# ysig/diff-mining

Measured on AMD Instinct MI355X. Metric: typicality-scored images/sec/node (512px, 10 t×2 prompts), higher is better.
Workload: dtype f16

## Files before the change

diff-mining_amd/build.py:

```python
from __future__ import annotations

import hashlib
import os
import subprocess
import sys
import time
from concurrent.futures import ThreadPoolExecutor

HERE = os.path.dirname(os.path.abspath(__file__))
CSRC = os.path.join(HERE, "csrc")
OBJ = os.path.join(CSRC, "build")
LIBDIR = os.path.join(HERE, "lib")
LIB = os.path.join(LIBDIR, "libdm_engine.so")
SOURCES = ["igemm.hip", "igemm_pers.hip", "igemm_pers_ln.hip", "igemm_pers_part.hip", "igemm_pers_ws.hip", "igemm_ws.hip", "igemm_pers_sc.hip", "igemm_sc.hip", "igemm_pers_tr.hip", "igemm_pers_up.hip", "igemm_ko.hip", "igemm_ln.hip", "igemm64.hip", "igemm_splitk.hip", "attention.hip", "attention_pipe.hip", "attention_qk32.hip", "attention_d160.hip", "attention_pp.hip", "attention_pipe80.hip", "attention_cross.hip", "resize.hip", "norm.hip", "misc.hip", "conv_out.hip", "vae.hip", "clip.hip", "f32_gemm.hip", "f32_ops.hip", "unet_f32.hip", "probe_peak.hip", "engine.hip"]
HEADERS = [os.path.join(CSRC, "dm_kernels.h"), os.path.join(CSRC, "f32_kernels.h"), os.path.join(CSRC, "arena.h"), os.path.join(CSRC, "igemm_tile.h"), os.path.join(CSRC, "igemm_pers_tile.h"), os.path.join(os.path.dirname(HERE), "include", "dm_engine.h")]
FLAGS = ["--offload-arch=gfx950", "-O3", "-std=c++17", "-fPIC", "-ffp-contract=off", "-Wno-unused-result",
         "-mllvm", "-amdgpu-mfma-vgpr-form=1"]


def _hipcc() -> str:
    for c in (os.environ.get("HIPCC"), "/opt/rocm/bin/hipcc", "hipcc"):
        if c and (os.path.isabs(c) and os.path.exists(c) or not os.path.isabs(c)):
            return c
    raise RuntimeError("hipcc not found")


def _read(path: str) -> bytes:
    with open(path, "rb") as f:
        return f.read()


_hipcc_id_cache = {}


def _hipcc_id(hipcc: str) -> bytes:
    if hipcc not in _hipcc_id_cache:
        r = subprocess.run([hipcc, "--version"], capture_output=True, text=True)
        _hipcc_id_cache[hipcc] = (r.stdout + r.stderr).encode()
    return _hipcc_id_cache[hipcc]


def tu_digest(src: str, hipcc: str) -> str:
    h = hashlib.sha256()
    h.update(_read(os.path.join(CSRC, src)))
    for hd in HEADERS:
        h.update(hd.encode())
        h.update(_read(hd))
    h.update(" ".join(FLAGS).encode())
    h.update(_hipcc_id(hipcc))
    return h.hexdigest()


def _stamp(obj: str) -> str:
    return obj + ".sha256"


def _tu_stale(src: str, obj: str, hipcc: str) -> bool:
    if not os.path.exists(obj) or not os.path.exists(_stamp(obj)):
        return True
    return _read(_stamp(obj)).decode().strip() != tu_digest(src, hipcc)


def build(force: bool = False, verbose: bool = False) -> str:
    os.makedirs(OBJ, exist_ok=True)
    os.makedirs(LIBDIR, exist_ok=True)
    hipcc = _hipcc()
    force = force or os.environ.get("DM_BUILD_FORCE", "0") not in ("", "0")
    t0 = time.time()
    jobs = []
    for src in SOURCES:
        o = os.path.join(OBJ, src.replace(".hip", ".o"))
        if force or _tu_stale(src, o, hipcc):
            jobs.append((src, o, [hipcc] + FLAGS + ["-c", os.path.join(CSRC, src), "-o", o]))

    def run(cmd):
        if verbose:
            print(" ".join(cmd), file=sys.stderr)
        r = subprocess.run(cmd, capture_output=True, text=True)
        if r.returncode != 0:
            raise RuntimeError("hipcc failed:\n" + " ".join(cmd) + "\n" + r.stdout + r.stderr)

    def compile_one(job):
        src, o, cmd = job
        if os.path.exists(_stamp(o)):
            os.remove(_stamp(o))
        run(cmd)
        with open(_stamp(o), "w") as f:
            f.write(tu_digest(src, hipcc) + "\n")
    with ThreadPoolExecutor(max_workers=min(8, os.cpu_count() or 1)) as ex:
        list(ex.map(compile_one, jobs))
    objs = [os.path.join(OBJ, s.replace(".hip", ".o")) for s in SOURCES]
    link_digest = hashlib.sha256("".join(_read(_stamp(o)).decode() for o in objs).encode()).hexdigest()
    linked = False
    if force or jobs or not os.path.exists(LIB) or not os.path.exists(_stamp(LIB)) or _read(_stamp(LIB)).decode().strip() != link_digest:
        run([hipcc, "--offload-arch=gfx950", "-shared", "-fPIC", "-o", LIB] + objs)
        with open(_stamp(LIB), "w") as f:
            f.write(link_digest + "\n")
        linked = True
    print(f"dm_engine build: compiled {len(jobs)}/{len(SOURCES)} TUs"
          f"{' (' + ', '.join(j[0] for j in jobs) + ')' if jobs and len(jobs) < len(SOURCES) else ''}, "
          f"{'linked' if linked else 'link up to date'} {os.path.relpath(LIB, os.path.dirname(HERE))} "
          f"[{link_digest[:12]}] in {time.time() - t0:.1f} s{' (forced)' if force else ''}", file=sys.stderr, flush=True)
    return LIB


if __name__ == "__main__":
    print(build(force="--force" in sys.argv, verbose="-v" in sys.argv))
```

diff-mining_amd/csrc/attention.hip:

```cpp
#include "dm_kernels.h"
#include <cstdlib>

namespace dm {

typedef _Float16 half8 __attribute__((ext_vector_type(8)));
typedef _Float16 half4 __attribute__((ext_vector_type(4)));
typedef float floatx4 __attribute__((ext_vector_type(4)));
typedef unsigned int u32x4 __attribute__((ext_vector_type(4)));
typedef unsigned int u32x2 __attribute__((ext_vector_type(2)));

namespace {

constexpr int KT = 64;
constexpr int NT = 256;
constexpr float RESCALE_THR = 8.0f;

__device__ __attribute__((aligned(256))) unsigned char g_attn_zero[256];
typedef const __attribute__((address_space(1))) void* gptr_t;
typedef __attribute__((address_space(3))) void* lptr_t;

template <int D, int QF>
__global__ __launch_bounds__(NT, (D > 80 ? 1 : 2))
void attn_kernel(AttnParams p) {
    constexpr int DP = ((D + 31) / 32) * 32, DV = ((D + 15) / 16) * 16;
// ... 142 lines not shown
            mx = __builtin_fmaxf(mx, __shfl_xor(mx, 32));
            if constexpr (FOLD) {
                float ps = 0.f;
                if (first || __builtin_amdgcn_ballot_w64(mx > RESCALE_THR) != 0ull) {
                    const float delta = first ? mx : __builtin_fmaxf(mx, 0.f);
                    const float alpha = first ? 0.f : __builtin_amdgcn_exp2f(-delta);
                    m_run[jq] += delta;
                    if (!LONES) l_run[jq] *= alpha;
#pragma unroll
                    for (int e = 0; e < EF; ++e) oacc[e][jq] *= alpha;
                    if (lg == LGX) {
                        const f16 mh = (f16)m_run[jq];
                        const f16 ml = (f16)(m_run[jq] - (float)mh);
                        qf[jq][SX][0] = -mh; qf[jq][SX][1] = -ml;
                    }
#pragma unroll
                    for (int f = 0; f < 4; ++f)
#pragma unroll
                        for (int r = 0; r < 4; ++r) {
                            const float pv = __builtin_amdgcn_exp2f(sacc[f][jq][r] - delta);
                            if (!LONES) ps += pv;
                            pb[jq][f >> 1][(f & 1) * 4 + r] = (f16)pv;
                        }
                } else {
#pragma unroll
                    for (int f = 0; f < 4; ++f)
#pragma unroll
                        for (int r = 0; r < 4; ++r) {
                            const float pv = __builtin_amdgcn_exp2f(sacc[f][jq][r]);
                            if (!LONES) ps += pv;
                            pb[jq][f >> 1][(f & 1) * 4 + r] = (f16)pv;
                        }
                }
                if (!LONES) l_run[jq] += ps;
            } else {
                const float mxs = mx * sc;
                if (__builtin_amdgcn_ballot_w64(mxs > m_run[jq] + RESCALE_THR) != 0ull) {
                    const float m_new = __builtin_fmaxf(m_run[jq], mxs);
                    const float alpha = __builtin_amdgcn_exp2f(m_run[jq] - m_new);
                    m_run[jq] = m_new;
                    l_run[jq] *= alpha;
#pragma unroll
                    for (int e = 0; e < EF; ++e) oacc[e][jq] *= alpha;
                }
                const float m_use = m_run[jq];
                float ps = 0.f;
#pragma unroll
                for (int f = 0; f < 4; ++f)
#pragma unroll
                    for (int r = 0; r < 4; ++r) {
                        const float pv = __builtin_amdgcn_exp2f(__builtin_fmaf(sacc[f][jq][r], sc, -m_use));
                        ps += pv;
                        pb[jq][f >> 1][(f & 1) * 4 + r] = (f16)pv;
                    }
                l_run[jq] += ps;
            }
        }
        constexpr int NB = (EF <= 5) ? 1 : 2;
#pragma unroll
        for (int bt = 0; bt < NB; ++bt) {
            u32x2 vraw[2 / NB][EF][2];
#pragma unroll
            for (int s2 = 0; s2 < 2 / NB; ++s2)
#pragma unroll
                for (int e = 0; e < EF; ++e)
#pragma unroll
                    for (int hh = 0; hh < 2; ++hh) {
                        const int ss = bt * (2 / NB) + s2;
                        const unsigned a = (unsigned)(size_t)(kt + voff[e] + (2 * ss + hh) * vstep[e]);
                        asm volatile("ds_read_b64_tr_b16 %0, %1" : "=v"(vraw[s2][e][hh]) : "v"(a) : "memory");
                    }
            asm volatile("s_waitcnt lgkmcnt(0)" ::: "memory");
            __builtin_amdgcn_sched_barrier(0);
#pragma unroll
            for (int s2 = 0; s2 < 2 / NB; ++s2)
#pragma unroll
                for (int e = 0; e < EF; ++e) {
                    const int ss = bt * (2 / NB) + s2;
                    half8 va;
                    __builtin_memcpy(&va, &vraw[s2][e][0], 8);
                    __builtin_memcpy(reinterpret_cast<char*>(&va) + 8, &vraw[s2][e][1], 8);
#pragma unroll
                    for (int jq = 0; jq < QF; ++jq)
                        oacc[e][jq] = __builtin_amdgcn_mfma_f32_16x16x32_f16(va, pb[jq][ss], oacc[e][jq], 0, 0, 0);
                }
        }
    };

    const int ntiles = (p.Tk + KT - 1) / KT;
    auto compute_tile = [&](int cur, int k0) __attribute__((always_inline)) {
        if (k0 + 64 > p.Tk) compute(cur, k0, true, k0 == 0); else compute(cur, k0, false, k0 == 0);
    };
    issue(0, 0);
    for (int t = 0; t < ntiles; ++t) {
        const int cur = t & 1;
        asm volatile("s_waitcnt vmcnt(0)" ::: "memory");
        __syncthreads();
        if (t + 1 < ntiles) issue(cur ^ 1, (t + 1) * KT);
        compute_tile(cur, t * KT);
    }

#pragma unroll
    for (int jq = 0; jq < QF; ++jq) {
        float l;
        if constexpr (LONES) {
            l = __shfl(oacc[EX][jq][0], (VLX << 4) | l15);
        } else {
            l = l_run[jq];
            l += __shfl_xor(l, 16);
            l += __shfl_xor(l, 32);
        }
        const float inv = 1.0f / l;
        const int q = q0 + 16 * jq + l15;
        if (q >= p.Tq) continue;
#pragma unroll
        for (int e = 0; e < EF; ++e) {
            const int d = 16 * e + 4 * lg;
            if (d < D) {
                const half4 o = half4{(f16)(oacc[e][jq][0] * inv), (f16)(oacc[e][jq][1] * inv),
                                      (f16)(oacc[e][jq][2] * inv), (f16)(oacc[e][jq][3] * inv)};
                *reinterpret_cast<half4*>(Ob + (size_t)q * p.ldo + d) = o;
            }
        }
    }
}

template <int D, int QF>
hipError_t launch_t(const AttnParams& p, hipStream_t s) {
    constexpr int QBLK = 64 * QF;
    dim3 grid((p.Tq + QBLK - 1) / QBLK, p.heads, p.B), block(NT);
    const size_t lds = 2 * (2 * (size_t)KT * D * 2 + 64);
    static std::atomic<uint64_t> attr_seen{0};
    if (first_use_on_device(attr_seen)) {
        (void)hipFuncSetAttribute((const void*)attn_kernel<D, QF>, hipFuncAttributeMaxDynamicSharedMemorySize, (int)lds);
    }
    launch_timed((attn_kernel<D, QF>), grid, block, lds, s, p);
    return hipGetLastError();
}

}

hipError_t launch_attention_pipe(const AttnParams& p, hipStream_t s);
bool attention_pipe_supports(const AttnParams& p);
hipError_t launch_attention_pipe80(const AttnParams& p, hipStream_t s);
bool attention_pipe80_supports(const AttnParams& p);
hipError_t launch_attention_cross(const AttnParams& p, hipStream_t s);
bool attention_cross_supports(const AttnParams& p);
hipError_t launch_attention_d160(const AttnParams& p, hipStream_t s);
bool attention_d160_supports(const AttnParams& p);
hipError_t launch_attention_d160_cross(const AttnParams& p, hipStream_t s);
bool attention_d160_cross_supports(const AttnParams& p);
hipError_t launch_attention_qk32(const AttnParams& p, hipStream_t s);
bool attention_qk32_supports(const AttnParams& p);
hipError_t launch_attention_pp(const AttnParams& p, int variant, hipStream_t s);
bool attention_pp_supports(const AttnParams& p);

hipError_t launch_attention(const AttnParams& p, hipStream_t s) {
    if (p.Tq <= 0 || p.Tk <= 0 || p.B <= 0) return hipErrorInvalidValue;
    if (option(OPT_ATTN_CROSS) && attention_cross_supports(p)) return launch_attention_cross(p, s);
    if (option(OPT_ATTN_CROSS) && attention_d160_cross_supports(p)) return launch_attention_d160_cross(p, s);
    const int pipe = option(OPT_ATTN_PIPE);
    if (p.q_mod > 0) {
        switch (p.D) { case 40: return launch_t<40, 2>(p, s); case 80: return launch_t<80, 2>(p, s); case 160: return launch_t<160, 2>(p, s); default: return hipErrorInvalidValue; }
    }
    if ((pipe == 10 || pipe == 12) && attention_pp_supports(p)) return launch_attention_pp(p, pipe, s);
    if (pipe == 5 && attention_qk32_supports(p)) return launch_attention_qk32(p, s);
#ifdef DM_ATTN_PP_ABLATE
    if (pipe >= 4 && pipe != 9 && attention_pp_supports(p)) return launch_attention_pp(p, pipe, s);
#endif
    if (pipe == 1 && p.Tk >= 8192 && attention_pp_supports(p) && (long long)((p.Tq + 383) / 384) * 384 * 50 <= 51LL * p.Tq)
        return launch_attention_pp(p, 12, s);
    if (pipe == 1 && attention_qk32_supports(p)) return launch_attention_qk32(p, s);
    if (pipe && attention_pipe_supports(p)) return launch_attention_pipe(p, s);
    if ((pipe == 1 || pipe >= 3) && attention_pipe80_supports(p)) return launch_attention_pipe80(p, s);
    if ((pipe == 1 || pipe == 5) && attention_d160_supports(p)) return launch_attention_d160(p, s);
    switch (p.D) {
        case 40: return launch_t<40, 2>(p, s);
        case 80: return launch_t<80, 2>(p, s);
        case 160: return launch_t<160, 2>(p, s);
        default: return hipErrorInvalidValue;
    }
}

}
```

diff-mining_amd/csrc/engine.hip:

```cpp
#include "../../include/dm_engine.h"
#include "dm_kernels.h"
#include "arena.h"

#include <cmath>
#include <cstdio>
#include <cstdlib>
#include <cstring>
#include <map>
#include <string>
#include <vector>

using namespace dm;

namespace {

thread_local std::string g_create_error;
}
namespace dm { thread_local LaunchTimer* g_launch_timer = nullptr; }
namespace {

constexpr int NB = 4;
const int BOC[NB] = {320, 640, 1280, 1280};
constexpr int LAYERS = 2;
constexpr int CTX_DIM = 768;
// ... 1055 lines not shown
        F.free(h);
        DM_TRY(F.alloc(&a, 1, 1, M, CL_H));
        if (!dry) DM_HIP(e, launch_clip_attention(qkv.p, n, CL_T, CL_HEADS, a.p, s));
        F.free(qkv);
        DM_TRY(F.dense(L.o, a, nullptr, &x, EPI_PLAIN, &x1));
        F.free(a); F.free(x);
        DM_TRY(F.layernorm(L.ln2, x1, &h));
        DM_TRY(F.dense(L.fc1, h, nullptr, nullptr, EPI_PLAIN, &f));
        F.free(h);
        if (!dry) DM_HIP(e, launch_quick_gelu(f.p, (long long)M * CL_F, s));
        DM_TRY(F.dense(L.fc2, f, nullptr, &x1, EPI_PLAIN, &x2));
        F.free(f); F.free(x1);
        x = x2;
    }
    Tensor y;
    DM_TRY(F.layernorm(c.final_ln, x, &y));
    F.free(x);
    if (!dry) {
        if (out16) DM_HIP(e, hipMemcpyAsync(out16, y.p, (size_t)M * CL_H * sizeof(f16), hipMemcpyDeviceToDevice, s));
        if (out32) DM_HIP(e, launch_f16_to_f32(y.p, out32, (long long)M * CL_H, s));
    }
    F.free(y);
    return 0;
}

void drop_graphs(dm_engine* e) {
    for (auto& g : e->graphs) (void)hipGraphExecDestroy(g.exec);
    e->graphs.clear();
}

template <class RunFn>
int ensure_arena_for(dm_engine* e, hipStream_t s, const std::vector<long long>& key, RunFn run_dry) {
    size_t need;
    if (e->opt_epoch != options_epoch()) {
        if (!e->graphs.empty()) { DM_HIP(e, hipStreamSynchronize(s)); drop_graphs(e); }
        e->arena_need.clear(); e->graph_seen.clear();
        e->opt_epoch = options_epoch();
    }
    auto it = e->arena_need.find(key);
    if (it != e->arena_need.end()) need = it->second;
    else {
        e->arena.reset((size_t)1 << 60, true);
        char* keep = e->arena_base;
        e->arena_base = nullptr;
        int rc = run_dry();
        e->arena_base = keep;
        if (rc) return rc;
        need = e->arena.peak;
        e->arena_need[key] = need;
        ++e->n_dry_runs;
    }
    if (need > e->arena_cap) {
        DM_HIP(e, hipStreamSynchronize(s));
        drop_graphs(e);
        if (e->arena_base) DM_HIP(e, hipFree(e->arena_base));
        e->arena_base = nullptr; e->arena_cap = 0;
        const size_t cap = need + (need >> 4);
        DM_MALLOC(e, &e->arena_base, cap);
        e->arena_cap = cap;
    }
    e->arena.reset(e->arena_cap, false);
    return 0;
}

std::vector<long long> fwd_key(const FwdArgs& A) {
    return {0, A.B, A.H, A.W, A.n_cond, A.up_ft_index, A.add_noise ? 1 : 0, A.loss ? 1 : 0, A.pred ? 1 : 0, A.feat ? 1 : 0,
            A.feat_mean ? 1 : 0, option(OPT_LN_FOLD), option(OPT_IGEMM_SPLITK), option(OPT_LN_INKERNEL), option(OPT_GN_FOLD), option(OPT_SC_FOLD), option(OPT_FF_FOLD), option(OPT_UP_FOLD), option(OPT_Q_ONCE), option(OPT_GN_EPI), option(OPT_CONV_OUT_ROWS), option(OPT_GN_SKIP)};
}

int ensure_arena(dm_engine* e, const FwdArgs& A, hipStream_t s) {
    return ensure_arena_for(e, s, fwd_key(A), [&]() { return run_forward(e, A, s, true); });
}

int reserve_prompts(dm_engine* e, int n_prompts, hipStream_t s) {
    if (n_prompts <= e->kv_capacity) return 0;
    int cap = e->kv_capacity > 0 ? 2 * e->kv_capacity : 16;
    if (cap < n_prompts) cap = n_prompts;
    DM_HIP(e, hipStreamSynchronize(s));
    drop_graphs(e);
    for (int l = 0; l < e->n_tf; ++l) {
        if (e->kv_cache[l]) DM_HIP(e, hipFree(e->kv_cache[l]));
        e->kv_cache[l] = nullptr;
        DM_MALLOC(e, &e->kv_cache[l], (size_t)cap * CTX_LEN * 2 * e->tfs[l]->c * sizeof(f16));
    }
    e->kv_capacity = cap;
    e->n_prompts = 0;
    return 0;
}

int run_forward_graphed(dm_engine* e, const FwdArgs& A, hipStream_t s) {
    if (!option(OPT_GRAPH) || e->prof || s == nullptr) return run_forward(e, A, s, false);
    std::vector<long long> key = fwd_key(A);
    for (const void* q : {A.x, (const void*)A.x_index, A.eps, (const void*)A.t, (const void*)A.slots, (const void*)A.loss,
                          (const void*)A.pred, (const void*)A.feat, (const void*)A.feat_mean, (const void*)s})
        key.push_back((long long)(size_t)q);
    for (long long v : {(long long)A.latent_f32, (long long)A.out_stride, (long long)A.out_off, (long long)A.ensemble, (long long)e->n_prompts})
        key.push_back(v);
    for (int o = 0; o < OPT_COUNT; ++o) key.push_back(option((Option)o));
    for (auto& g : e->graphs)
        if (g.key == key) {
            g.stamp = ++e->graph_stamp;
            ++e->n_graph_launches;
            DM_HIP(e, hipGraphLaunch(g.exec, s));
            return 0;
        }
    if (e->graph_seen.size() > 256) e->graph_seen.clear();
    if (e->graph_seen[key]++ == 0) return run_forward(e, A, s, false);
    hipGraph_t graph = nullptr;
    DM_HIP(e, hipStreamBeginCapture(s, hipStreamCaptureModeThreadLocal));
    const int rc = run_forward(e, A, s, false);
    const hipError_t ec = hipStreamEndCapture(s, &graph);
    if (rc) { if (graph) (void)hipGraphDestroy(graph); return rc; }
    if (ec != hipSuccess || !graph) DM_FAIL(e, "hipStreamEndCapture failed: %s", hipGetErrorString(ec));
    hipGraphExec_t exec = nullptr;
    const hipError_t ei = hipGraphInstantiate(&exec, graph, nullptr, nullptr, 0);
    (void)hipGraphDestroy(graph);
    if (ei != hipSuccess) DM_FAIL(e, "hipGraphInstantiate failed: %s", hipGetErrorString(ei));
    if (e->graphs.size() >= 8) {
        size_t old = 0;
        for (size_t i = 1; i < e->graphs.size(); ++i) if (e->graphs[i].stamp < e->graphs[old].stamp) old = i;
        (void)hipGraphExecDestroy(e->graphs[old].exec);
        e->graphs.erase(e->graphs.begin() + old);
    }
    e->graphs.push_back({key, exec, ++e->graph_stamp});
    ++e->n_graph_captures; ++e->n_graph_launches;
    DM_HIP(e, hipGraphLaunch(exec, s));
    return 0;
}

int max_chunk(int h, int w) {
    const long long px = (long long)h * w;
    static long long budget = -1;
    if (budget < 0) { const char* e = getenv("DM_CHUNK"); budget = e ? atoll(e) : 160; if (budget < 1) budget = 1; }
    long long b = (budget * 4096) / px;
    if (b < 1) b = 1;
    return (int)b;
}

}

namespace dm {

namespace {
struct OptDef { const char* name; const char* env; int def; };
const OptDef kOpts[OPT_COUNT] = {
    {"igemm_big", "DM_IGEMM_BIG", -1}, {"igemm_splitk", "DM_IGEMM_SPLITK", 1},
    {"ln_fold", "DM_LN_FOLD", 1}, {"attn_pipe", "DM_ATTN_PIPE", 1}, {"igemm_tail", "DM_IGEMM_TAIL", 1}, {"attn_cross", "DM_ATTN_CROSS", 1}, {"ln_stats_g", "DM_LN_STATS_G", 1}, {"igemm_exp", "DM_IGEMM_EXP", 0}, {"ln_inkernel", "DM_LN_INKERNEL", 1}, {"graph", "DM_GRAPH", 0}, {"gn_fold", "DM_GN_FOLD", 1}, {"sc_fold", "DM_SC_FOLD", 1}, {"ff_fold", "DM_FF_FOLD", 1}, {"tap_reuse", "DM_TAP_REUSE", 1}, {"up_fold", "DM_UP_FOLD", 1}, {"q_once", "DM_Q_ONCE", 1}, {"gn_epi", "DM_GN_EPI", 1}, {"conv_out_rows", "DM_CONV_OUT_ROWS", 1}, {"gn_skip", "DM_GN_SKIP", 1},
};
static bool option_value_ok(int i, int value) {
    if (i == OPT_ATTN_PIPE) {
#ifdef DM_ATTN_PP_ABLATE
        return value >= 0 && value <= 51;
#else
        return value == 0 || value == 1 || value == 2 || value == 3 || value == 5 || value == 9 || value == 10 || value == 12;
#endif
    }
    if (i == OPT_IGEMM_BIG) return value >= -1 && value <= 2;
    return value >= 0 && value <= 2;
}
std::atomic<int> g_opt[OPT_COUNT];
std::atomic<int> g_opt_init{0};
std::atomic<unsigned> g_opt_epoch{1};
void opts_init() {
    if (g_opt_init.load() == 2) return;
    int expect = 0;
    if (g_opt_init.compare_exchange_strong(expect, 1)) {
        for (int i = 0; i < OPT_COUNT; ++i) {
            const char* e = getenv(kOpts[i].env);
            int v = e ? atoi(e) : kOpts[i].def;
            if (e && !option_value_ok(i, v)) {
                fprintf(stderr, "dm_engine: %s=%s is not a value of option \"%s\"; using the default %d\n", kOpts[i].env, e, kOpts[i].name, kOpts[i].def);
                v = kOpts[i].def;
            }
            g_opt[i] = v;
        }
        g_opt_init = 2;
    } else while (g_opt_init.load() != 2) {}
}
}

int option(Option o) { opts_init(); return g_opt[o].load(std::memory_order_relaxed); }
unsigned options_epoch() { return g_opt_epoch.load(std::memory_order_relaxed); }

void fold_upconv_weights(const f16* w, int cout, int cin, f16* out) {
    static const int lo[2][2] = {{0, 1}, {0, 2}}, hi[2][2] = {{0, 2}, {1, 2}};
    for (int py = 0; py < 2; ++py)
        for (int px = 0; px < 2; ++px) {
            f16* o = out + (size_t)(py * 2 + px) * cout * 4 * cin;
            for (int co = 0; co < cout; ++co)
                for (int a = 0; a < 2; ++a)
                    for (int b = 0; b < 2; ++b)
                        for (int ci = 0; ci < cin; ++ci) {
                            const f16* k9 = w + ((size_t)co * cin + ci) * 9;
                            float acc = 0.f;
                            for (int dy = lo[py][a]; dy <= hi[py][a]; ++dy)
                                for (int dx = lo[px][b]; dx <= hi[px][b]; ++dx) acc += (float)k9[dy * 3 + dx];
                            o[(size_t)co * 4 * cin + (size_t)(a * 2 + b) * cin + ci] = (f16)acc;
                        }
        }
}
int get_option(const char* name, int* value) {
    opts_init();
    for (int i = 0; i < OPT_COUNT; ++i)
        if (name && value && !strcmp(name, kOpts[i].name)) { *value = g_opt[i].load(); return 0; }
    return 1;
}
int set_option(const char* name, int value) {
    opts_init();
    for (int i = 0; i < OPT_COUNT; ++i)
        if (name && !strcmp(name, kOpts[i].name)) {
            if (!option_value_ok(i, value)) return 2;
            if (g_opt[i].exchange(value) != value) g_opt_epoch.fetch_add(1);
            return 0;
        }
    return 1;
}

}

int dm_get_option_up_fold() { return dm::option(dm::OPT_UP_FOLD); }

extern "C" {

const char* dm_version(void) { return "dm_engine 0.2 (gfx950; igemm 128x320 / persistent 256x320 x64 mfma_f32_16x16x32_f16, LDS-DMA)"; }

int dm_scheduler_alphas_cumprod(int n, float beta_start, float beta_end, float* out) {
    if (n < 2 || !out) return 1;
    host_alphas_cumprod(n, beta_start, beta_end, out);
    return 0;
}

int dm_timestep_sinusoid(int t, int dim, float* out) {
    if (dim < 2 || (dim & 1) || !out) return 1;
    host_sinusoid(t, dim, out);
    return 0;
}

const char* dm_last_error(dm_engine* e) { return e ? e->err.c_str() : g_create_error.c_str(); }

int dm_engine_create(int device, dm_engine** out) {
    if (!out) return 1;
    int n = 0;
    hipError_t r = hipGetDeviceCount(&n);
    if (r != hipSuccess || n <= 0) { g_create_error = "no HIP device available (the engine has no CPU fallback)"; return 1; }
    if (device < 0 || device >= n) { g_create_error = "bad device index"; return 1; }
    r = hipSetDevice(device);
    if (r != hipSuccess) { g_create_error = hipGetErrorString(r); return 1; }
    dm_engine* e = new dm_engine();
    e->device = device;
    *out = e;
    return 0;
}

void dm_engine_destroy(dm_engine* e) {
    if (!e) return;
    (void)hipSetDevice(e->device);
    (void)hipDeviceSynchronize();
    if (e->wslab) (void)hipFree(e->wslab);
    if (e->vslab) (void)hipFree(e->vslab);
    if (e->cslab) (void)hipFree(e->cslab);
    if (e->arena_base) (void)hipFree(e->arena_base);
    if (e->tile_ctr) (void)hipFree(e->tile_ctr);
    if (e->slot_scratch) (void)hipFree(e->slot_scratch);
    if (e->sin_table) (void)hipFree(e->sin_table);
    if (e->sa_tab) (void)hipFree(e->sa_tab);
    if (e->sb_tab) (void)hipFree(e->sb_tab);
    if (e->sa32_tab) (void)hipFree(e->sa32_tab);
    if (e->sb32_tab) (void)hipFree(e->sb32_tab);
    for (auto p : e->kv_cache) if (p) (void)hipFree(p);
    for (auto& g : e->graphs) (void)hipGraphExecDestroy(g.exec);
    for (auto& ev : e->prof_ev) for (hipEvent_t h : ev.pairs) (void)hipEventDestroy(h);
    for (auto ev : e->ev_pool) (void)hipEventDestroy(ev);
    delete e;
}

int dm_engine_load_weight(dm_engine* e, const char* name, const void* host_ptr, int dtype, const int64_t* shape, int ndim) {
    if (!e || !name || !host_ptr || !shape) return 1;
    if (e->finalized) DM_FAIL(e, "load_weight after finalize");
    HostTensor t;
    t.shape.assign(shape, shape + ndim);
    const size_t n = t.numel();
    t.data.resize(n);
    if (dtype == DM_F16) memcpy(t.data.data(), host_ptr, n * 2);
    else if (dtype == DM_F32) { const float* f = (const float*)host_ptr; for (size_t i = 0; i < n; ++i) t.data[i] = (f16)f[i]; }
    else DM_FAIL(e, "unsupported dtype %d for %s", dtype, name);
    e->host[name] = std::move(t);
    return 0;
}

int dm_engine_finalize(dm_engine* e) {
    if (!e) return 1;
    if (e->finalized) return 0;
    DM_HIP(e, hipSetDevice(e->device));
    Packer P{e, {}};
    std::vector<f16> tw, tb;
    e->n_tf = 0; e->tfs.clear();
    {
        HostTensor* w = P.get("conv_in.weight", {BOC[0], 4, 3, 3});
        if (!w) return 1;
        std::vector<f16> pk((size_t)BOC[0] * 64, (f16)0.f);
        for (int co = 0; co < BOC[0]; ++co)
            for (int k = 0; k < 36; ++k) pk[(size_t)co * 64 + k] = w->data[(size_t)co * 36 + k];
        e->conv_in.w = as_ptr(P.put(pk.data(), pk.size() * 2));
        e->conv_in.cin = 64; e->conv_in.cout = BOC[0]; e->conv_in.k = 1;
        DM_TRY(pack_bias(P, "conv_in", BOC[0], &e->conv_in.b));
    }
    DM_TRY(pack_dense(P, "time_embedding.linear_1", TEMB, BOC[0], false, true, &e->time1));
// ... 823 lines not shown
```

Baseline: 59.56.

## Add D=40 attention kernel with 64 queries per wave and make it default

Adds a new D=40 flash-attention kernel where each wave handles two 32-query slices (64 queries), so every K/V tile loaded into LDS is reused across twice as many queries. It uses a 3-stage LDS ring, transposed LDS reads for V, and software-interleaved exp, score MFMA and PV MFMA phases. The default attn_pipe=1 path now picks this kernel instead of the qk32 one, and option value 6 selects it explicitly. In exchange it holds more accumulator registers per wave and launches fewer blocks, which can lower occupancy or leave fewer blocks for short query lengths.

```diff
diff --git a/diff-mining_amd/build.py b/diff-mining_amd/build.py
--- a/diff-mining_amd/build.py
+++ b/diff-mining_amd/build.py
@@ -12,7 +12,7 @@
 OBJ = os.path.join(CSRC, "build")
 LIBDIR = os.path.join(HERE, "lib")
 LIB = os.path.join(LIBDIR, "libdm_engine.so")
-SOURCES = ["igemm.hip", "igemm_pers.hip", "igemm_pers_ln.hip", "igemm_pers_part.hip", "igemm_pers_ws.hip", "igemm_ws.hip", "igemm_pers_sc.hip", "igemm_sc.hip", "igemm_pers_tr.hip", "igemm_pers_up.hip", "igemm_ko.hip", "igemm_ln.hip", "igemm64.hip", "igemm_splitk.hip", "attention.hip", "attention_pipe.hip", "attention_qk32.hip", "attention_d160.hip", "attention_pp.hip", "attention_pipe80.hip", "attention_cross.hip", "resize.hip", "norm.hip", "misc.hip", "conv_out.hip", "vae.hip", "clip.hip", "f32_gemm.hip", "f32_ops.hip", "unet_f32.hip", "probe_peak.hip", "engine.hip"]
+SOURCES = ["igemm.hip", "igemm_pers.hip", "igemm_pers_ln.hip", "igemm_pers_part.hip", "igemm_pers_ws.hip", "igemm_ws.hip", "igemm_pers_sc.hip", "igemm_sc.hip", "igemm_pers_tr.hip", "igemm_pers_up.hip", "igemm_ko.hip", "igemm_ln.hip", "igemm64.hip", "igemm_splitk.hip", "attention.hip", "attention_pipe.hip", "attention_qk32.hip", "attention_qk64.hip", "attention_d160.hip", "attention_pp.hip", "attention_pipe80.hip", "attention_cross.hip", "resize.hip", "norm.hip", "misc.hip", "conv_out.hip", "vae.hip", "clip.hip", "f32_gemm.hip", "f32_ops.hip", "unet_f32.hip", "probe_peak.hip", "engine.hip"]
 HEADERS = [os.path.join(CSRC, "dm_kernels.h"), os.path.join(CSRC, "f32_kernels.h"), os.path.join(CSRC, "arena.h"), os.path.join(CSRC, "igemm_tile.h"), os.path.join(CSRC, "igemm_pers_tile.h"), os.path.join(os.path.dirname(HERE), "include", "dm_engine.h")]
 FLAGS = ["--offload-arch=gfx950", "-O3", "-std=c++17", "-fPIC", "-ffp-contract=off", "-Wno-unused-result",
          "-mllvm", "-amdgpu-mfma-vgpr-form=1"]
diff --git a/diff-mining_amd/csrc/attention.hip b/diff-mining_amd/csrc/attention.hip
--- a/diff-mining_amd/csrc/attention.hip
+++ b/diff-mining_amd/csrc/attention.hip
@@ -318,6 +318,8 @@
 bool attention_d160_cross_supports(const AttnParams& p);
 hipError_t launch_attention_qk32(const AttnParams& p, hipStream_t s);
 bool attention_qk32_supports(const AttnParams& p);
+hipError_t launch_attention_qk64(const AttnParams& p, hipStream_t s);
+bool attention_qk64_supports(const AttnParams& p);
 hipError_t launch_attention_pp(const AttnParams& p, int variant, hipStream_t s);
 bool attention_pp_supports(const AttnParams& p);
 
@@ -331,15 +333,16 @@
     }
     if ((pipe == 10 || pipe == 12) && attention_pp_supports(p)) return launch_attention_pp(p, pipe, s);
     if (pipe == 5 && attention_qk32_supports(p)) return launch_attention_qk32(p, s);
+    if (pipe == 6 && attention_qk64_supports(p)) return launch_attention_qk64(p, s);
 #ifdef DM_ATTN_PP_ABLATE
     if (pipe >= 4 && pipe != 9 && attention_pp_supports(p)) return launch_attention_pp(p, pipe, s);
 #endif
     if (pipe == 1 && p.Tk >= 8192 && attention_pp_supports(p) && (long long)((p.Tq + 383) / 384) * 384 * 50 <= 51LL * p.Tq)
         return launch_attention_pp(p, 12, s);
-    if (pipe == 1 && attention_qk32_supports(p)) return launch_attention_qk32(p, s);
+    if (pipe == 1 && attention_qk64_supports(p)) return launch_attention_qk64(p, s);
     if (pipe && attention_pipe_supports(p)) return launch_attention_pipe(p, s);
     if ((pipe == 1 || pipe >= 3) && attention_pipe80_supports(p)) return launch_attention_pipe80(p, s);
-    if ((pipe == 1 || pipe == 5) && attention_d160_supports(p)) return launch_attention_d160(p, s);
+    if ((pipe == 1 || pipe == 5 || pipe == 6) && attention_d160_supports(p)) return launch_attention_d160(p, s);
     switch (p.D) {
         case 40: return launch_t<40, 2>(p, s);
         case 80: return launch_t<80, 2>(p, s);
diff --git a/diff-mining_amd/csrc/attention_qk64.hip b/diff-mining_amd/csrc/attention_qk64.hip
--- /dev/null
+++ b/diff-mining_amd/csrc/attention_qk64.hip
@@ -0,0 +1,360 @@
+#include "dm_kernels.h"
+
+namespace dm {
+
+typedef _Float16 half8 __attribute__((ext_vector_type(8)));
+typedef _Float16 half4 __attribute__((ext_vector_type(4)));
+typedef _Float16 half2v __attribute__((ext_vector_type(2)));
+typedef float floatx4 __attribute__((ext_vector_type(4)));
+typedef float floatx16 __attribute__((ext_vector_type(16)));
+typedef unsigned int u32x2 __attribute__((ext_vector_type(2)));
+
+namespace {
+
+constexpr int D = 40;
+constexpr int KT = 64;
+constexpr int NT = 256;
+constexpr int QS = 32;
+constexpr int NS = 2;
+constexpr int QW = NS * QS;
+constexpr float RESCALE_THR = 8.0f;
+constexpr int RS = 96;
+constexpr int TILE = KT * RS;
+constexpr int KOFF = 0, VOFF = TILE + 32;
+constexpr int STAGE = 2 * (TILE + 32);
+constexpr int NSTG = 3;
+constexpr int EF = 3;
+
+__device__ __attribute__((aligned(16))) const unsigned short g_kconst64[8] = {0x3C00, 0x3C00, 0, 0, 0, 0, 0, 0};
+__device__ __attribute__((aligned(16))) const unsigned short g_vconst64[8] = {0x3C00, 0, 0, 0, 0, 0, 0, 0};
+typedef const __attribute__((address_space(1))) void* gptr_t;
+typedef __attribute__((address_space(3))) void* lptr_t;
+
+#define PIN(x) asm volatile("" : "+v"(x))
+
+__device__ __forceinline__ float vmax2(float a, float b) { float r; asm("v_max_f32 %0, %1, %2" : "=v"(r) : "v"(a), "v"(b)); return r; }
+__device__ __forceinline__ float vmax3(float a, float b, float c) { float r; asm("v_max3_f32 %0, %1, %2, %3" : "=v"(r) : "v"(a), "v"(b), "v"(c)); return r; }
+__device__ __forceinline__ void vmax2x2(float& x, float& y, float a0, float a1, float b0, float b1) {
+    asm("v_max_f32 %0, %2, %3\n\tv_max_f32 %1, %4, %5" : "=&v"(x), "=&v"(y) : "v"(a0), "v"(a1), "v"(b0), "v"(b1));
+}
+__device__ __forceinline__ void vmax3x2(float& x, float& y, float a0, float a1, float b0, float b1) {
+    asm("v_max3_f32 %0, %0, %2, %3\n\tv_max3_f32 %1, %1, %4, %5" : "+v"(x), "+v"(y) : "v"(a0), "v"(a1), "v"(b0), "v"(b1));
+}
+__device__ __forceinline__ void swap16(unsigned& a, unsigned& b) {
+    const auto r = __builtin_amdgcn_permlane16_swap(a, b, false, false);
+    a = r[0]; b = r[1];
+}
+
+template <int OFF>
+__device__ __forceinline__ void tr_read(u32x2& out, unsigned base) {
+    asm volatile("ds_read_b64_tr_b16 %0, %1 offset:%2" : "=v"(out) : "v"(base), "n"(OFF) : "memory");
+}
+
+__global__ __launch_bounds__(NT, 2)
+void attn_qk64_kernel(AttnParams p) {
+    extern __shared__ __attribute__((aligned(16))) char smem[];
+
+    const int tid = threadIdx.x;
+    const int lane = tid & 63;
+    const int wid = __builtin_amdgcn_readfirstlane(tid >> 6);
+    const int l15 = lane & 15;
+    const int lg = lane >> 4;
+    const int l31 = lane & 31;
+    const int hh5 = lane >> 5;
+    const int nqb = (p.Tq + 4 * QW - 1) / (4 * QW);
+    int v;
+    {
+        const int nblk = gridDim.x, bid = blockIdx.x;
+        const int q = nblk >> 3, r = nblk & 7;
+        const int xcd = bid & 7, loc = bid >> 3;
+        v = (xcd < r ? xcd * (q + 1) : r * (q + 1) + (xcd - r) * q) + loc;
+    }
+    const int qblk = v % nqb;
+    const int bh = v / nqb;
+    const int h = bh % p.heads;
+    const int b = bh / p.heads;
+    const int q0 = qblk * (4 * QW) + wid * QW;
+    int kvb = p.kv_slot ? p.kv_slot[b] : (p.slot_div > 0 ? b / p.slot_div : b);
+    if (p.n_slots > 0) kvb = kvb < 0 ? 0 : (kvb < p.n_slots ? kvb : p.n_slots - 1);
+
+    const f16* Qb = p.Q + (size_t)b * p.bsq + h * D;
+    const f16* Kb = p.K + (size_t)kvb * p.bsk + h * D;
+    const f16* Vb = p.V + (size_t)kvb * p.bsv + h * D;
+    f16* Ob = p.O + (size_t)b * p.bso + h * D;
+
+    const float sc = p.scale * 1.44269504088896340736f;
+    half8 qf[NS][3];
+#pragma unroll
+    for (int j = 0; j < NS; ++j) {
+        int q = q0 + QS * j + l31;
+        q = q < p.Tq ? q : p.Tq - 1;
+#pragma unroll
+        for (int s = 0; s < 3; ++s) {
+            const int d = 16 * s + 8 * hh5;
+            if (d < D) qf[j][s] = *reinterpret_cast<const half8*>(Qb + (size_t)q * p.ldq + d);
+            else qf[j][s] = half8{0, 0, 0, 0, 0, 0, 0, 0};
+#pragma unroll
+            for (int k = 0; k < 8; ++k) qf[j][s][k] = (f16)((float)qf[j][s][k] * sc);
+        }
+    }
+
+    const f16* gsrc[3];
+    int ginc[3];
+#pragma unroll
+    for (int i = 0; i < 3; ++i) {
+        const int j = wid + 4 * i;
+        const bool isv = j >= 6;
+        const int jj = isv ? j - 6 : j;
+        const int idx = jj * 64 + lane;
+        const int row = idx / 6, pch = idx - row * 6;
+        const int key = isv ? ((row & ~20) | ((row & 4) << 2) | ((row & 16) >> 2)) : row;
+        const int ch = isv ? pch : (pch ^ ((row >> 3) & 1));
+        const int ld = isv ? p.ldv : p.ldk;
+        if (ch < 5) { gsrc[i] = (isv ? Vb : Kb) + (size_t)key * ld + ch * 8; ginc[i] = KT * ld; }
+        else { gsrc[i] = reinterpret_cast<const f16*>(isv ? g_vconst64 : g_kconst64); ginc[i] = 0; }
+    }
+    auto piece_is_v = [&](int i) __attribute__((always_inline)) { return wid + 4 * i >= 6; };
+    auto piece = [&](int i, int kst, int vst) __attribute__((always_inline)) {
+        const int j = wid + 4 * i;
+        char* dst = smem + ((j >= 6) ? vst * STAGE + VOFF + (j - 6) * 1024 : kst * STAGE + KOFF + j * 1024);
+        __builtin_amdgcn_global_load_lds((gptr_t)gsrc[i], (lptr_t)dst, 16, 0, 0);
+        gsrc[i] += ginc[i];
+    };
+
+    const char* kbase = smem + l31 * RS + 16 * (hh5 ^ ((lane >> 3) & 1));
+    const unsigned vbase = (unsigned)(size_t)(smem + (4 * (lg & 1) + 16 * (lg >> 1) + (l15 >> 2)) * RS + 8 * (l15 & 3));
+
+    floatx4 oacc[NS][EF][2];
+#pragma unroll
+    for (int j = 0; j < NS; ++j)
+#pragma unroll
+        for (int e = 0; e < EF; ++e)
+#pragma unroll
+            for (int jq = 0; jq < 2; ++jq) oacc[j][e][jq] = floatx4{0, 0, 0, 0};
+    float m_run[NS] = {0.f, 0.f};
+
+    floatx16 S[NS][2];
+    unsigned pk[NS][2][8];
+
+    auto rescale = [&](const int j, const float mxl, bool first) __attribute__((always_inline)) {
+        float mown = mxl;
+        PIN(mown);
+        const float mx = __builtin_fmaxf(mown, __shfl_xor(mown, 32));
+        const float delta = first ? mx : __builtin_fmaxf(mx, 0.f);
+        const float alpha = first ? 0.f : __builtin_amdgcn_exp2f(-delta);
+        m_run[j] += delta;
+        const float alpha_x = __shfl_xor(alpha, 16);
+        const float a0 = (lg & 1) ? alpha_x : alpha, a1 = (lg & 1) ? alpha : alpha_x;
+#pragma unroll
+        for (int e = 0; e < EF; ++e) { oacc[j][e][0] *= a0; oacc[j][e][1] *= a1; }
+        if (hh5 == 1) {
+            const f16 mh = (f16)m_run[j];
+            const f16 ml = (f16)(m_run[j] - (float)mh);
+            qf[j][2][0] = -mh; qf[j][2][1] = -ml;
+        }
+#pragma unroll
+        for (int mb = 0; mb < 2; ++mb)
+#pragma unroll
+            for (int r = 0; r < 16; ++r) S[j][mb][r] -= delta;
+    };
+    auto exp_slice = [&](const int j, int i) __attribute__((always_inline)) {
+        const int mb = i >> 3, pp = i & 7;
+        const half2v hv = half2v{(f16)__builtin_amdgcn_exp2f(S[j][mb][2 * pp]), (f16)__builtin_amdgcn_exp2f(S[j][mb][2 * pp + 1])};
+        unsigned u;
+        __builtin_memcpy(&u, &hv, 4);
+        PIN(u);
+        pk[j][mb][pp] = u;
+    };
+    auto score_mfma = [&](const int j, const half8 (&kf)[3][2], int m) __attribute__((always_inline)) {
+        const int s = m >> 1, mb = m & 1;
+        S[j][mb] = __builtin_amdgcn_mfma_f32_32x32x16_f16(kf[s][mb], qf[j][s], S[j][mb], 0, 0, 0);
+        PIN(S[j][mb]);
+    };
+    auto pv_mfma = [&](const int j, const u32x2 (&vraw)[2][EF][2], int m) __attribute__((always_inline)) {
+        const int ss = m / 6, e = (m % 6) >> 1, jq = (m & 1) ^ (DM_MFMA_SNAKE ? (e & 1) : 0);
+        half8 va, pbv;
+        __builtin_memcpy(&va, &vraw[ss][e][0], 8);
+        __builtin_memcpy(reinterpret_cast<char*>(&va) + 8, &vraw[ss][e][1], 8);
+        __builtin_memcpy(&pbv, &pk[j][ss][4 * jq], 16);
+        oacc[j][e][jq] = __builtin_amdgcn_mfma_f32_16x16x32_f16(va, pbv, oacc[j][e][jq], 0, 0, 0);
+        PIN(oacc[j][e][jq]);
+    };
+    auto max_step = [&](const int j, float (&mx)[4], int o) __attribute__((always_inline)) {
+        const int c = o & 1, r = 8 * c + 2 * (o >> 1);
+        if (o < 2) vmax2x2(mx[c], mx[2 + c], S[j][0][r], S[j][0][r + 1], S[j][1][r], S[j][1][r + 1]);
+        else vmax3x2(mx[c], mx[2 + c], S[j][0][r], S[j][0][r + 1], S[j][1][r], S[j][1][r + 1]);
+    };
+
+    const int ntiles = p.Tk / KT;
+
+#pragma unroll
+    for (int i = 0; i < 3; ++i) if (!piece_is_v(i)) piece(i, 0, 0);
+    asm volatile("s_waitcnt vmcnt(0)" ::: "memory");
+    __syncthreads();
+#pragma unroll
+    for (int i = 0; i < 3; ++i) piece(i, 1, 0);
+#pragma unroll
+    for (int i = 0; i < 3; ++i) piece(i, 2, 1);
+    {
+        half8 kf[3][2];
+#pragma unroll
+        for (int s = 0; s < 3; ++s)
+#pragma unroll
+            for (int mb = 0; mb < 2; ++mb) kf[s][mb] = *reinterpret_cast<const half8*>(kbase + KOFF + 32 * s + mb * 32 * RS);
+#pragma unroll
+        for (int j = 0; j < NS; ++j) {
+#pragma unroll
+            for (int mb = 0; mb < 2; ++mb)
+#pragma unroll
+                for (int r = 0; r < 16; ++r) S[j][mb][r] = 0.f;
+#pragma unroll
+            for (int s = 0; s < 3; ++s)
+#pragma unroll
+                for (int mb = 0; mb < 2; ++mb) S[j][mb] = __builtin_amdgcn_mfma_f32_32x32x16_f16(kf[s][mb], qf[j][s], S[j][mb], 0, 0, 0);
+        }
+#pragma unroll
+        for (int j = 0; j < NS; ++j) {
+            float m = S[j][0][0];
+#pragma unroll
+            for (int mb = 0; mb < 2; ++mb)
+#pragma unroll
+                for (int r = 0; r < 16; ++r) m = __builtin_fmaxf(m, S[j][mb][r]);
+            rescale(j, m, true);
+        }
+    }
+
+    int s0 = 0;
+    auto iteration = [&](const bool next, const bool dma_k, const bool dma_v, const bool wait3) __attribute__((always_inline)) {
+        constexpr int KB = KOFF, VB = VOFF;
+        const int s1 = (s0 == NSTG - 1) ? 0 : s0 + 1;
+        const int s2 = (s1 == NSTG - 1) ? 0 : s1 + 1;
+        const char* kcur = kbase + s1 * STAGE;
+        const unsigned vcur = vbase + (unsigned)(s0 * STAGE);
+        if (wait3) asm volatile("s_waitcnt vmcnt(3)" ::: "memory"); else asm volatile("s_waitcnt vmcnt(0)" ::: "memory");
+        asm volatile("s_barrier" ::: "memory");
+        half8 kf[3][2];
+        u32x2 vraw[2][EF][2];
+        if (next) {
+#pragma unroll
+            for (int s = 0; s < 3; ++s)
+#pragma unroll
+                for (int mb = 0; mb < 2; ++mb) kf[s][mb] = *reinterpret_cast<const half8*>(kcur + KB + 32 * s + mb * 32 * RS);
+        }
+#pragma unroll
+        for (int i = 0; i < 16; ++i) {
+            exp_slice(0, i);
+            if (i == 2) { tr_read<VB + 0 + 0 * 8 * RS>(vraw[0][0][0], vcur); tr_read<VB + 0 + 1 * 8 * RS>(vraw[0][0][1], vcur); }
+            if (i == 4) { tr_read<VB + 32 + 0 * 8 * RS>(vraw[0][1][0], vcur); tr_read<VB + 32 + 1 * 8 * RS>(vraw[0][1][1], vcur); }
+            if (i == 6) { tr_read<VB + 64 + 0 * 8 * RS>(vraw[0][2][0], vcur); tr_read<VB + 64 + 1 * 8 * RS>(vraw[0][2][1], vcur); }
+            if (i == 8) { tr_read<VB + 0 + 4 * 8 * RS>(vraw[1][0][0], vcur); tr_read<VB + 0 + 5 * 8 * RS>(vraw[1][0][1], vcur); }
+            if (i == 10) { tr_read<VB + 32 + 4 * 8 * RS>(vraw[1][1][0], vcur); tr_read<VB + 32 + 5 * 8 * RS>(vraw[1][1][1], vcur); }
+            if (i == 12) { tr_read<VB + 64 + 4 * 8 * RS>(vraw[1][2][0], vcur); tr_read<VB + 64 + 5 * 8 * RS>(vraw[1][2][1], vcur); }
+            if (i == 9) { swap16(pk[0][0][0], pk[0][0][4]); swap16(pk[0][0][1], pk[0][0][5]); }
+            if (i == 11) { swap16(pk[0][0][2], pk[0][0][6]); swap16(pk[0][0][3], pk[0][0][7]); }
+            if (i & 1) __builtin_amdgcn_sched_barrier(0);
+        }
+#pragma unroll
+        for (int i = 0; i < 4; ++i) swap16(pk[0][1][i], pk[0][1][4 + i]);
+        __builtin_amdgcn_sched_barrier(0);
+        if (next) asm volatile("s_waitcnt lgkmcnt(12)" ::: "memory");
+        __builtin_amdgcn_sched_barrier(0);
+        if (next) {
+#pragma unroll
+            for (int mb = 0; mb < 2; ++mb)
+#pragma unroll
+                for (int r = 0; r < 16; ++r) S[0][mb][r] = 0.f;
+        }
+#pragma unroll
+        for (int m = 0; m < 6; ++m) {
+            if (next) score_mfma(0, kf, m);
+            exp_slice(1, 2 * m);
+            exp_slice(1, 2 * m + 1);
+            if (m == 4) { swap16(pk[1][0][0], pk[1][0][4]); swap16(pk[1][0][1], pk[1][0][5]); }
+            if (m == 5) { swap16(pk[1][0][2], pk[1][0][6]); swap16(pk[1][0][3], pk[1][0][7]); }
+            __builtin_amdgcn_sched_barrier(0);
+        }
+        asm volatile("s_waitcnt lgkmcnt(0)" ::: "memory");
+        __builtin_amdgcn_sched_barrier(0);
+        float mx0[4], mx1[4];
+#pragma unroll
+        for (int m = 0; m < 12; ++m) {
+            pv_mfma(0, vraw, m);
+            if (m < 2) { exp_slice(1, 12 + 2 * m); exp_slice(1, 13 + 2 * m); }
+            if (m >= 2 && m < 6) swap16(pk[1][1][m - 2], pk[1][1][m + 2]);
+            if (next && m >= 4) max_step(0, mx0, m - 4);
+            __builtin_amdgcn_sched_barrier(0);
+        }
+        if (next) {
+#pragma unroll
+            for (int mb = 0; mb < 2; ++mb)
+#pragma unroll
+                for (int r = 0; r < 16; ++r) S[1][mb][r] = 0.f;
+        }
+#pragma unroll
+        for (int m = 0; m < 6; ++m) {
+            if (next) score_mfma(1, kf, m);
+            if (m == 0 || m == 2 || m == 4) {
+                const int i = m >> 1;
+                if (piece_is_v(i) ? dma_v : dma_k) piece(i, s0, s2);
+            }
+            __builtin_amdgcn_sched_barrier(0);
+        }
+        if (next) {
+            const float mx = vmax2(vmax3(mx0[0], mx0[1], mx0[2]), mx0[3]);
+            if (__builtin_amdgcn_ballot_w64(mx > RESCALE_THR) != 0ull) rescale(0, mx, false);
+        }
+        __builtin_amdgcn_sched_barrier(0);
+#pragma unroll
+        for (int m = 0; m < 12; ++m) {
+            pv_mfma(1, vraw, m);
+            if (next && m >= 4) max_step(1, mx1, m - 4);
+            __builtin_amdgcn_sched_barrier(0);
+        }
+        if (next) {
+            const float mx = vmax2(vmax3(mx1[0], mx1[1], mx1[2]), mx1[3]);
+            if (__builtin_amdgcn_ballot_w64(mx > RESCALE_THR) != 0ull) rescale(1, mx, false);
+        }
+        s0 = s1;
+    };
+
+    for (int t = 0; t < ntiles - 3; ++t) iteration(true, true, true, true);
+    iteration(true, false, true, true);
+    iteration(true, false, false, false);
+    iteration(false, false, false, false);
+
+#pragma unroll
+    for (int j = 0; j < NS; ++j)
+#pragma unroll
+        for (int jq = 0; jq < 2; ++jq) {
+            const float l = __shfl(oacc[j][2][jq][0], (2 << 4) | l15);
+            const float inv = 1.0f / l;
+            const int q = q0 + QS * j + 16 * jq + l15;
+            if (q >= p.Tq) continue;
+#pragma unroll
+            for (int e = 0; e < EF; ++e) {
+                const int d = 16 * e + 4 * lg;
+                if (d < D) {
+                    const half4 o = half4{(f16)(oacc[j][e][jq][0] * inv), (f16)(oacc[j][e][jq][1] * inv),
+                                          (f16)(oacc[j][e][jq][2] * inv), (f16)(oacc[j][e][jq][3] * inv)};
+                    *reinterpret_cast<half4*>(Ob + (size_t)q * p.ldo + d) = o;
+                }
+            }
+        }
+}
+
+}
+
+bool attention_qk64_supports(const AttnParams& p) {
+    return p.D == 40 && p.Tk >= 256 && (p.Tk % 128) == 0 && p.q_mod == 0;
+}
+
+hipError_t launch_attention_qk64(const AttnParams& p, hipStream_t s) {
+    if (!attention_qk64_supports(p)) return hipErrorInvalidValue;
+    constexpr int QBLK = 4 * QW;
+    dim3 grid(((p.Tq + QBLK - 1) / QBLK) * p.heads * p.B), block(NT);
+    const size_t lds = NSTG * (size_t)STAGE;
+    launch_timed(attn_qk64_kernel, grid, block, lds, s, p);
+    return hipGetLastError();
+}
+
+}
diff --git a/diff-mining_amd/csrc/engine.hip b/diff-mining_amd/csrc/engine.hip
--- a/diff-mining_amd/csrc/engine.hip
+++ b/diff-mining_amd/csrc/engine.hip
@@ -1231,7 +1231,7 @@
 #ifdef DM_ATTN_PP_ABLATE
         return value >= 0 && value <= 51;
 #else
-        return value == 0 || value == 1 || value == 2 || value == 3 || value == 5 || value == 9 || value == 10 || value == 12;
+        return value == 0 || value == 1 || value == 2 || value == 3 || value == 5 || value == 6 || value == 9 || value == 10 || value == 12;
 #endif
     }
     if (i == OPT_IGEMM_BIG) return value >= -1 && value <= 2;
```

Result: faster. 60.56 (median of 6 runs) (+1.7%).
